# Ricardo-Ping/ChaoRec

Measured on AMD Instinct MI355X. Metric: GCN edges/sec + full-rank users-scored/sec, dim=64, higher is better.
Workload: dtype f32

## Files before the change

### chaorec_amd/csrc/score_prefilter.hpp

```cpp
#pragma once

typedef __bf16 bf16x8 __attribute__((ext_vector_type(8)));

union Frag16 {
  uint4 u;
  bf16x8 v;
};

__device__ __forceinline__ uint32_t bf16_rne_bits(float f) {
  const uint32_t b = __float_as_uint(f);
  return (b + 0x7FFFu + ((b >> 16) & 1u)) >> 16;
}
__device__ __forceinline__ float bf16_ceil_pos(float x) {
  const uint32_t b = __float_as_uint(x);
  return __uint_as_float(((b >> 16) + ((b & 0xFFFFu) ? 1u : 0u)) << 16);
}
__device__ __forceinline__ uint32_t bf16_pack2(float lo, float hi) {
  return bf16_rne_bits(lo) | (bf16_rne_bits(hi) << 16);
}
__device__ __forceinline__ uint4 bf16_pack8(const float4 a, const float4 b) {
  return make_uint4(bf16_pack2(a.x, a.y), bf16_pack2(a.z, a.w), bf16_pack2(b.x, b.y), bf16_pack2(b.z, b.w));
}

template <int CTRL, int ROW_MASK, bool BOUND>
// ... 819 lines not shown
      int tt = split + (kSweepStage * s0 + i) * splits;
      if (tt >= n_tiles) tt = n_tiles - 1;
      pre[p] = make_uint4(0u, 0u, 0u, 0u);
      if (i < kSweepStage) pre[p] = P.packed[(size_t)tt * (FR * 64) + w];
    }
  };
  auto stash = [&](int buf) __attribute__((always_inline)) {
#pragma unroll
    for (int p = 0; p < PER; ++p) {
      const int e = threadIdx.x + p * 64 * kSweepWaves;
      if (e < kSweepStage * FR * 64) (&stage[buf][0][0])[e] = pre[p];
    }
  };
  const int n_mine = split < n_tiles ? (n_tiles - split + splits - 1) / splits : 0;
  const int n_stages = (n_mine + kSweepStage - 1) / kSweepStage;
  int next_nb = 0;
  if (n_stages > 0) {
    fetch(0);
    stash(0);
    if constexpr (CLS) next_nb = __builtin_amdgcn_readfirstlane(__float_as_int(pre_nb));
  }
  __syncthreads();
  int s0 = 0;
  while (s0 < n_stages) {
    if constexpr (CLS) {
      cur_nb = next_nb;
      rescale(__int_as_float(cur_nb));
    }
    for (;;) {
      const int buf = s0 & 1;
      if (s0 + 1 < n_stages) fetch(s0 + 1);
#pragma unroll
      for (int i = 0; i < kSweepStage; ++i) {
        const int seq = kSweepStage * s0 + i;
        const int t = split + seq * splits;
        if (t < n_tiles) {
          uint4 a[FR];
#pragma unroll
          for (int q = 0; q < FR; ++q) a[q] = stage[buf][i][q * 64 + lane];
          consume(a, t, seq);
        }
      }
      if (s0 + 1 < n_stages) {
        stash(buf ^ 1);
        if constexpr (CLS) next_nb = __builtin_amdgcn_readfirstlane(__float_as_int(pre_nb));
      }
      __syncthreads();
      ++s0;
      if (s0 >= n_stages) break;
      if constexpr (CLS) {
        if (next_nb != cur_nb) break;
      }
    }
  }
#pragma unroll
  for (int b = 0; b < UB; ++b) {
    if constexpr (kSweepPark > 0) {
#pragma unroll
      for (int c0 = 0; c0 < kSweepPark; c0 += 4) {
        if (c0 < cnt[b]) {
          uint4 q;
          q.x = park_s[wv][b][c0][lane], q.y = park_s[wv][b][c0 + 1][lane];
          q.z = park_s[wv][b][c0 + 2][lane], q.w = park_s[wv][b][c0 + 3][lane];
          *reinterpret_cast<uint4 *>(mine[b] + c0) = q;
        }
      }
    }
    const int64_t uc = (ublock0 + b) * 32 + ur;
    if (uc < n_act) {
      const int64_t u = P.user_map ? (int64_t)P.user_map[uc] : uc;
      P.cand_cnt[((size_t)split * P.n_users + u) * 2 + h] = cnt[b];
    }
  }
}

template <int D>
__device__ __forceinline__ float exact_score(const float *__restrict__ urow, const float *__restrict__ irow) {
  float acc = 0.f;
  const float4 *i0 = reinterpret_cast<const float4 *>(irow), *i1 = reinterpret_cast<const float4 *>(irow + D / 2);
  const float4 *u0 = reinterpret_cast<const float4 *>(urow), *u1 = reinterpret_cast<const float4 *>(urow + D / 2);
#pragma unroll
  for (int q = 0; q < D / 8; ++q) {
    const float4 a = i0[q], b = i1[q], x = u0[q], y = u1[q];
    acc = __fmaf_rn(x.x, a.x, acc);
    acc = __fmaf_rn(y.x, b.x, acc);
    acc = __fmaf_rn(x.y, a.y, acc);
    acc = __fmaf_rn(y.y, b.y, acc);
    acc = __fmaf_rn(x.z, a.z, acc);
    acc = __fmaf_rn(y.z, b.z, acc);
    acc = __fmaf_rn(x.w, a.w, acc);
    acc = __fmaf_rn(y.w, b.w, acc);
  }
  return acc;
}

__device__ __forceinline__ float dpp_quad_rot(float v) {
  return __int_as_float(__builtin_amdgcn_update_dpp(0, __float_as_int(v), 0x93 , 0xF, 0xF, false));
}
template <int D>
__device__ __forceinline__ float exact_scores_64(const float *__restrict__ item_emb, int64_t i0, int64_t n_items,
                                                 const float (&ua)[D / 8], const float (&ub)[D / 8], int lane) {
  constexpr int G = 4, CPI = 16, SEG = D / 8;
  const int l = lane % G, g = lane / G;
  auto load_rows = [&](float (&a)[SEG], float (&b)[SEG], int pass) __attribute__((always_inline)) {
    const int64_t item = min(i0 + pass * CPI + g, n_items - 1);
    const float *row = item_emb + (size_t)item * D + 4 * l;
#pragma unroll
    for (int i = 0; i < SEG; i += 4) {
      const float4 x = reinterpret_cast<const float4 *>(row + 4 * i)[0];
      const float4 y = reinterpret_cast<const float4 *>(row + D / 2 + 4 * i)[0];
      a[i] = x.x, a[i + 1] = x.y, a[i + 2] = x.z, a[i + 3] = x.w;
      b[i] = y.x, b[i + 1] = y.y, b[i + 2] = y.z, b[i + 3] = y.w;
    }
  };
  float sc = 0.f;
  float a[SEG], b[SEG];
  load_rows(a, b, 0);
#pragma unroll
  for (int it = 0; it < G; ++it) {
    float ca[SEG], cb[SEG];
#pragma unroll
    for (int i = 0; i < SEG; ++i) ca[i] = a[i], cb[i] = b[i];
    if (it + 1 < G) load_rows(a, b, it + 1);
    float acc = 0.f;
#pragma unroll
    for (int seg = 0; seg < SEG; ++seg) {
      float t = acc;
#pragma unroll
      for (int i = 4 * (seg / G); i < 4 * (seg / G) + 4; ++i) {
        t = __fmaf_rn(ua[i], ca[i], t);
        t = __fmaf_rn(ub[i], cb[i], t);
      }
      if (l == seg % G) acc = t;
      if (seg + 1 < SEG) {
        const float nx = dpp_quad_rot(acc);
        if (l == (seg + 1) % G) acc = nx;
      }
    }
    const float moved = __shfl(acc, (lane % CPI) * G + G - 1, 64);
    if (lane / CPI == it) sc = moved;
  }
  return sc;
}

template <int NR>
__device__ __forceinline__ uint64_t kth_largest_key(const uint64_t (&k)[NR], int rank) {
  uint32_t T = 0;
  for (int bit = 31; bit >= 0; --bit) {
    const uint32_t candv = T | (1u << bit);
    int c = 0;
#pragma unroll
    for (int r = 0; r < NR; ++r) c += __popcll(__ballot(k[r] != 0ull && (uint32_t)(k[r] >> 32) >= candv));
    if (c >= rank) T = candv;
  }
  int gt = 0, eq = 0;
#pragma unroll
  for (int r = 0; r < NR; ++r) {
    gt += __popcll(__ballot(k[r] != 0ull && (uint32_t)(k[r] >> 32) > T));
    eq += __popcll(__ballot(k[r] != 0ull && (uint32_t)(k[r] >> 32) == T));
  }
  const int need = rank - gt;
  uint32_t L = 0;
  if (eq > need) {
    for (int bit = 31; bit >= 0; --bit) {
      const uint32_t candv = L | (1u << bit);
      int c = 0;
#pragma unroll
      for (int r = 0; r < NR; ++r)
        c += __popcll(__ballot(k[r] != 0ull && (uint32_t)(k[r] >> 32) == T && (uint32_t)k[r] >= candv));
      if (c >= need) L = candv;
    }
  }
  return ((uint64_t)T << 32) | (uint64_t)L;
}

__device__ __forceinline__ void sort64_desc(uint64_t &e, int lane) {
#pragma unroll
  for (int k = 2; k <= 64; k <<= 1) {
#pragma unroll
    for (int j = k >> 1; j > 0; j >>= 1) {
      const uint64_t p = shfl_xor_u64(e, j);
      const bool lower = (lane & j) == 0;
      const bool desc = (k == 64) ? true : ((lane & k) == 0);
      const uint64_t mx = e > p ? e : p, mn = e > p ? p : e;
      e = (lower == desc) ? mx : mn;
    }
  }
}

constexpr int kPfHistLds = 1024;
constexpr int kPfSelHist = 128;


__device__ __forceinline__ int wave_scan_add(int x) {
  x += dpp_or0<0x111, 0xF, true>(x);
  x += dpp_or0<0x112, 0xF, true>(x);
  x += dpp_or0<0x114, 0xF, true>(x);
  x += dpp_or0<0x118, 0xF, true>(x);
  x += dpp_or0<0x142, 0xA, false>(x);
  x += dpp_or0<0x143, 0xC, false>(x);
  return x;
}
__device__ __forceinline__ int wave_scan_max(int x) {
  x = max(x, dpp_or0<0x111, 0xF, true>(x));
  x = max(x, dpp_or0<0x112, 0xF, true>(x));
  x = max(x, dpp_or0<0x114, 0xF, true>(x));
  x = max(x, dpp_or0<0x118, 0xF, true>(x));
  x = max(x, dpp_or0<0x142, 0xA, false>(x));
  x = max(x, dpp_or0<0x143, 0xC, false>(x));
  return x;
}
__device__ __forceinline__ float dpp_prev_lane(float v) {
  return __int_as_float(__builtin_amdgcn_update_dpp(0, __float_as_int(v), 0x111 , 0xF, 0xF, false));
}

__device__ __forceinline__ uint32_t lane_select(uint32_t a, uint32_t b, uint64_t m) {
  uint32_t r;
  asm("v_cndmask_b32 %0, %1, %2, %3" : "=v"(r) : "v"(a), "v"(b), "s"(m));
  return r;
}
__device__ __forceinline__ uint64_t lane_select64(uint64_t a, uint64_t b, uint64_t m) {
  return ((uint64_t)lane_select((uint32_t)(a >> 32), (uint32_t)(b >> 32), m) << 32) | lane_select((uint32_t)a, (uint32_t)b, m);
}
struct PermAddr {
  int x0, x1, x2, x3, x4, x5, rev;
  template <int I>
  __device__ __forceinline__ int x() const {
    if constexpr (I == 0) return x0;
    else if constexpr (I == 1) return x1;
    else if constexpr (I == 2) return x2;
    else if constexpr (I == 3) return x3;
    else if constexpr (I == 4) return x4;
    else return x5;
  }
};
__device__ __forceinline__ PermAddr perm_addr(int lane) {
  PermAddr a;
  a.x0 = (lane ^ 1) << 2, a.x1 = (lane ^ 2) << 2, a.x2 = (lane ^ 4) << 2, a.x3 = (lane ^ 8) << 2;
  a.x4 = (lane ^ 16) << 2, a.x5 = (lane ^ 32) << 2, a.rev = (63 - lane) << 2;
  return a;
}
__device__ __forceinline__ uint64_t permute64(uint64_t v, int addr) {
  const uint32_t lo = (uint32_t)__builtin_amdgcn_ds_bpermute(addr, (int)(uint32_t)v);
  const uint32_t hi = (uint32_t)__builtin_amdgcn_ds_bpermute(addr, (int)(uint32_t)(v >> 32));
  return ((uint64_t)hi << 32) | lo;
}
__device__ __forceinline__ void compare_exchange(uint64_t &e, uint64_t p, uint64_t keepmax) {
  const uint64_t gt = __ballot(p > e);
  e = lane_select64(e, p, ~(gt ^ keepmax));
}
constexpr uint64_t keepmax_mask(int k, int j, bool all_desc) {
  uint64_t m = 0;
  for (int lane = 0; lane < 64; ++lane) {
    const bool lower = (lane & j) == 0, desc = all_desc || (lane & k) == 0;
    if (lower == desc) m |= 1ull << lane;
  }
  return m;
}
template <int LOGJ>
__device__ __forceinline__ void merge_stages(uint64_t &e, const PermAddr &pa) {
  compare_exchange(e, permute64(e, pa.template x<LOGJ>()), keepmax_mask(64, 1 << LOGJ, true));
  if constexpr (LOGJ > 0) merge_stages<LOGJ - 1>(e, pa);
}
template <int LOGK, int LOGJ>
__device__ __forceinline__ void sort_stages(uint64_t &e, const PermAddr &pa) {
  compare_exchange(e, permute64(e, pa.template x<LOGJ>()), keepmax_mask(1 << LOGK, 1 << LOGJ, LOGK == 6));
  if constexpr (LOGJ > 0) sort_stages<LOGK, LOGJ - 1>(e, pa);
  else if constexpr (LOGK < 6) sort_stages<LOGK + 1, LOGK>(e, pa);
}
__device__ __forceinline__ void sort64_keys(uint64_t &e, const PermAddr &pa) { sort_stages<1, 0>(e, pa); }
__device__ __forceinline__ void merge128_keys(uint64_t &e0, uint64_t &e1, const PermAddr &pa) {
  const uint64_t r = permute64(e1, pa.rev);
  const uint64_t gt = __ballot(r > e0);
  const uint64_t hi = lane_select64(e0, r, gt), lo = lane_select64(r, e0, gt);
  e0 = hi;
  e1 = lo;
  merge_stages<5>(e0, pa);
  merge_stages<5>(e1, pa);
}
__device__ __forceinline__ void merge_block_keys(uint64_t &e0, uint64_t &e1, uint64_t b, const PermAddr &pa) {
  sort64_keys(b, pa);
  const uint64_t r = permute64(b, pa.rev);
  e1 = lane_select64(e1, r, __ballot(r > e1));
  merge_stages<5>(e1, pa);
  merge128_keys(e0, e1, pa);
}

__device__ __forceinline__ void take_block_keys(uint64_t &e0, uint64_t &e1, int &blocks, uint64_t cur, const PermAddr &pa) {
  if (blocks == 0) {
    sort64_keys(cur, pa);
    e0 = cur;
  } else if (blocks == 1) {
    sort64_keys(cur, pa);
    uint64_t a = e0, b = cur;
    merge128_keys(a, b, pa);
    e0 = a, e1 = b;
  } else {
    uint64_t a = e0, b = e1;
    merge_block_keys(a, b, cur, pa);
    e0 = a, e1 = b;
  }
  ++blocks;
}
__device__ __forceinline__ uint64_t key_of_rank(uint64_t e0, uint64_t e1, int rank) {
  const uint32_t lo0 = (uint32_t)__builtin_amdgcn_readlane((int)(uint32_t)e0, rank & 63);
  const uint32_t hi0 = (uint32_t)__builtin_amdgcn_readlane((int)(uint32_t)(e0 >> 32), rank & 63);
  const uint32_t lo1 = (uint32_t)__builtin_amdgcn_readlane((int)(uint32_t)e1, rank & 63);
  const uint32_t hi1 = (uint32_t)__builtin_amdgcn_readlane((int)(uint32_t)(e1 >> 32), rank & 63);
  return rank < 64 ? (((uint64_t)hi0 << 32) | lo0) : (((uint64_t)hi1 << 32) | lo1);
}

#ifndef CHAOREC_SEL_G
#define CHAOREC_SEL_G 4
#endif
constexpr int kSelG = CHAOREC_SEL_G;
template <int D>
__device__ __forceinline__ float chain_block(const float *__restrict__ item_emb, const uint32_t *cand_s, int base, int n_cand,
                                             const float (&ua)[D / (2 * kSelG)], const float (&ub)[D / (2 * kSelG)], int lane) {
  constexpr int G = kSelG, CPI = 64 / G, SEG = D / (2 * G);
  const int l = lane % G, g = lane / G;
  auto load_rows = [&](float (&a)[SEG], float (&b)[SEG], int c) __attribute__((always_inline)) {
    const float *row = item_emb + (size_t)cand_s[c] * D;
#pragma unroll
    for (int i = 0; i < SEG; i += 4) {
      const float4 x = reinterpret_cast<const float4 *>(row + SEG * l)[i / 4];
      const float4 y = reinterpret_cast<const float4 *>(row + D / 2 + SEG * l)[i / 4];
      a[i] = x.x, a[i + 1] = x.y, a[i + 2] = x.z, a[i + 3] = x.w;
      b[i] = y.x, b[i + 1] = y.y, b[i + 2] = y.z, b[i + 3] = y.w;
    }
  };
  float sc = 0.f;
  float a[SEG], b[SEG];
#pragma unroll
  for (int i = 0; i < SEG; ++i) a[i] = b[i] = 0.f;
  if (base + g < n_cand) load_rows(a, b, base + g);
  for (int it = 0; it < G; ++it) {
    if (base + it * CPI >= n_cand) break;
    float ca[SEG], cb[SEG];
#pragma unroll
    for (int i = 0; i < SEG; ++i) ca[i] = a[i], cb[i] = b[i];
    const int cn = base + (it + 1) * CPI + g;
    if (it + 1 < G && cn < n_cand) load_rows(a, b, cn);
    float acc = 0.f;
#pragma unroll
    for (int seg = 0; seg < G; ++seg) {
      float t = acc;
#pragma unroll
      for (int i = 0; i < SEG; ++i) {
        t = __fmaf_rn(ua[i], ca[i], t);
        t = __fmaf_rn(ub[i], cb[i], t);
      }
      if (l == seg) acc = t;
      if (seg + 1 < G) {
        const float nx = dpp_prev_lane(acc);
        if (l == seg + 1) acc = nx;
      }
    }
    const float moved = __shfl(acc, (lane % CPI) * G + G - 1, 64);
    if (lane / CPI == it) sc = moved;
  }
  return sc;
}

template <int D, int MAXC>
__device__ __forceinline__ void select_user(const PrefArgs &P, const int64_t u, int lane, int2 *meta_s, uint32_t *cand_s,
                                            uint32_t *hist_s, float *score_s) {
  const int K = P.K;
  const int n_lists = 2 * P.splits;
  const PermAddr pa = perm_addr(lane);

  const int listidx = (int)(((int64_t)(lane >> 1) * P.n_users + u) * 2 + (lane & 1));
  int c = 0;
  if (lane < n_lists) c = P.cand_cnt[listidx];
  float ua[D / (2 * kSelG)], ub[D / (2 * kSelG)];
  {
    const float *urow = P.user_emb + (size_t)u * D + (D / (2 * kSelG)) * (lane % kSelG);
#pragma unroll
    for (int i = 0; i < D / (2 * kSelG); i += 4) {
      const float4 x = reinterpret_cast<const float4 *>(urow)[i / 4], y = reinterpret_cast<const float4 *>(urow + D / 2)[i / 4];
      ua[i] = x.x, ua[i + 1] = x.y, ua[i + 2] = x.z, ua[i + 3] = x.w;
      ub[i] = y.x, ub[i + 1] = y.y, ub[i + 2] = y.z, ub[i + 3] = y.w;
    }
  }
  int64_t hb = 0, he = 0;
  if (P.hist_rowptr) {
    hb = P.hist_rowptr[u];
    he = P.hist_rowptr[u + 1];
  }
  const int deg = (int)(he - hb);
  const bool hist_lds = deg <= kPfSelHist;
  const float theta = P.theta[u];
  const bool overflow = __any(c > kPfCap);
  const int incl = wave_scan_add(c);
  const int total = __builtin_amdgcn_readlane(incl, 63);
  int why = overflow ? 1 : (total > MAXC ? 3 : 0);
  int n_cand = 0;
  if (why == 0) {
    int *owner_s = reinterpret_cast<int *>(score_s);
#pragma unroll 1
    for (int i = lane; i < total; i += 64) owner_s[i] = 0;
    meta_s[lane] = make_int2(incl - c, listidx);
    if (hist_lds) {
#pragma unroll 1
      for (int i = lane; i < deg; i += 64) hist_s[i] = (uint32_t)P.hist_col[hb + i];
    }
    __builtin_amdgcn_wave_barrier();
    if (c > 0) owner_s[incl - c] = lane + 1;
    __builtin_amdgcn_wave_barrier();
    int owner_carry = 0;
#pragma unroll 1
    for (int base = 0; base < total; base += 64) {
      const int e = base + lane;
      int own = e < total ? owner_s[e] : 0;
      own = max(wave_scan_max(own), owner_carry);
      owner_carry = __builtin_amdgcn_readlane(own, 63);
      uint32_t bits = 0, j0 = 0;
      if (e < total) {
        const int list = own - 1;
        const int2 m = meta_s[list];
        const uint32_t raw = P.cand[(size_t)m.y * kPfCap + (e - m.x)];
        bits = raw & 0xFFFFu;
        j0 = ((uint32_t)(list >> 1) + (raw >> 16) * (uint32_t)P.splits) * 32u + 4u * (uint32_t)(list & 1);
      }
      if (__any(bits != 0u && j0 + 32u > (uint32_t)P.n_items)) {
#pragma unroll 1
        for (int reg = 0; reg < 16; ++reg)
          if (j0 + (uint32_t)((reg & 3) + 8 * (reg >> 2)) >= (uint32_t)P.n_items) bits &= ~(1u << (15 - reg));
      }
      const int pc = __popc(bits);
      const int ex = wave_scan_add(pc);
      int slot = n_cand + ex - pc;
#pragma unroll 1
      while (__any(bits != 0u)) {
        if (bits) {
          const int bit = 31 - __clz(bits);
          bits &= ~(1u << bit);
          const int reg = 15 - bit;
          if (slot < MAXC) cand_s[slot] = j0 + (uint32_t)((reg & 3) + 8 * (reg >> 2));
          ++slot;
        }
      }
      n_cand += __builtin_amdgcn_readlane(ex, 63);
    }
    if (n_cand > MAXC) why = 3;
    __builtin_amdgcn_wave_barrier();
    if (P.perm && why == 0) {
#pragma unroll 1
      for (int i = lane; i < n_cand; i += 64) cand_s[i] = (uint32_t)P.perm[cand_s[i]];
      __builtin_amdgcn_wave_barrier();
    }
  }
  uint64_t e0 = 0ull, e1 = 0ull;
  if (why == 0) {
    auto in_hist = [&](uint32_t item) -> bool {
      int lo = 0, hi = deg;
      while (lo < hi) {
        const int mid = (lo + hi) >> 1;
        const uint32_t hv = hist_lds ? hist_s[mid] : (uint32_t)P.hist_col[hb + mid];
        if (hv < item) lo = mid + 1; else hi = mid;
      }
      return lo < deg && (hist_lds ? hist_s[lo] : (uint32_t)P.hist_col[hb + lo]) == item;
    };
    const uint32_t mord = f32_to_ord(P.mask_value);
    int valid = 0, above = 0, blocks = 0;
#pragma unroll 1
    for (int base = 0; base < n_cand; base += 64) {
      const float sc = chain_block<D>(P.item_emb, cand_s, base, n_cand, ua, ub, lane);
      const int idx = base + lane;
      uint64_t cur = 0ull;
      if (idx < n_cand) {
        const uint32_t item = cand_s[idx];
        if (deg == 0 || !in_hist(item)) cur = make_key(sc, item);
      }
      valid += __popcll(__ballot(cur != 0ull));
      above += __popcll(__ballot(cur != 0ull && (uint32_t)(cur >> 32) > mord));
      take_block_keys(e0, e1, blocks, cur, pa);
    }
    int n_keys = valid;
    if (deg > 0 && above < K) {
#pragma unroll 1
      for (int i0 = 0; i0 < deg; i0 += 64) {
        const int i = i0 + lane;
        take_block_keys(e0, e1, blocks, i < deg ? make_key(P.mask_value, hist_lds ? hist_s[i] : (uint32_t)P.hist_col[hb + i]) : 0ull, pa);
      }
      n_keys = valid + deg;
    }
    if (n_keys < K) why = 2;
    if (why == 0) {
      const uint64_t kth = key_of_rank(e0, e1, K - 1);
      if (kth == 0ull || !(ord_to_f32((uint32_t)(kth >> 32)) > theta)) why = 4;
      if (why == 0 && P.hint_out) {
        const int want = min(max(P.hint_rank, K), 128);
        const uint64_t hk = key_of_rank(e0, e1, min(want, n_keys) - 1);
        float t = nextafterf(ord_to_f32((uint32_t)(hk >> 32)), -INFINITY);
        if (n_keys < want) {
          const float s_k = ord_to_f32((uint32_t)(kth >> 32)), s_last = ord_to_f32((uint32_t)(hk >> 32));
          const float s_top = ord_to_f32((uint32_t)(key_of_rank(e0, e1, 0) >> 32));
          const float slope = n_keys > K ? (s_k - s_last) / (float)(n_keys - K) : (s_top - s_k) / (float)max(K - 1, 1);
          t -= slope * (float)(want - n_keys);
        }
        if (lane == 0) P.hint_out[u] = t;
      }
    }
  }
  if (lane == 0) {
    P.fail[u] = why;
    P.n_cand[u] = n_cand;
    if (why != 0) {
      if (P.retry_cnt) P.retry_list[atomicAdd(P.retry_cnt, 1)] = (int)u;
      else if (why == 3 && MAXC < kPfMaxCandWide && P.wide_cnt && n_cand <= kPfMaxCandWide && total <= kPfMaxCandWide)
        P.wide_list[atomicAdd(P.wide_cnt, 1)] = (int)u;
      else if ((why == 1 || why == 3) && P.reth_cnt) P.reth_list[atomicAdd(P.reth_cnt, 1)] = (int)u;
      else P.fb_list[atomicAdd(P.fb_cnt, 1)] = (int)u;
    }
  }
  if (why == 0 && lane < K) {
    const uint32_t item = 0xFFFFFFFFu - (uint32_t)(e0 & 0xFFFFFFFFull);
    P.out_idx[(size_t)u * K + lane] = (int64_t)item + P.id_offset;
    P.out_val[(size_t)u * K + lane] = ord_to_f32((uint32_t)(e0 >> 32));
  }
}

#ifndef CHAOREC_SEL_WAVES
#define CHAOREC_SEL_WAVES 4
#endif
template <int D, int MAXC>
__global__ __launch_bounds__(64, D > 64 ? 3 : (MAXC <= 512 ? CHAOREC_SEL_WAVES : 3)) void score_select_kernel_pf(const PrefArgs P) {
  __shared__ int2 meta_s[64];
  __shared__ uint32_t cand_s[MAXC];
  __shared__ uint32_t hist_s[kPfSelHist];
  __shared__ float score_s[MAXC];
  const int64_t n_act = P.n_active ? (int64_t)*P.n_active : P.n_users;
  if (n_act <= P.min_active) return;
#pragma unroll 1
  for (int64_t i = blockIdx.x; i < n_act; i += gridDim.x) {
    const int64_t u = P.user_map ? (int64_t)P.user_map[i] : i;
    int lane = threadIdx.x;
    asm volatile("" : "+v"(lane));
    select_user<D, MAXC>(P, u, lane, meta_s, cand_s, hist_s, score_s);
    __builtin_amdgcn_wave_barrier();
  }
}

constexpr int kPfRethTarget = 256;

template <int D>
__device__ __forceinline__ void rethreshold_user(const PrefArgs &P, const int64_t u, int lane, int2 *meta_s, uint32_t *cand_s,
                                                 uint32_t *hist_s, float *score_s) {
  constexpr int MAXC = kPfMaxCandWide;
  const int K = P.K;
  const int n_lists = 2 * P.splits;
  const PermAddr pa = perm_addr(lane);
  const int listidx = (int)(((int64_t)(lane >> 1) * P.n_users + u) * 2 + (lane & 1));
  int c_all = 0;
  if (lane < n_lists) c_all = P.cand_cnt[listidx];
  const int c = min(c_all, kPfCap);
  float ua[D / (2 * kSelG)], ub[D / (2 * kSelG)];
  {
    const float *urow = P.user_emb + (size_t)u * D + (D / (2 * kSelG)) * (lane % kSelG);
#pragma unroll
    for (int i = 0; i < D / (2 * kSelG); i += 4) {
      const float4 x = reinterpret_cast<const float4 *>(urow)[i / 4], y = reinterpret_cast<const float4 *>(urow + D / 2)[i / 4];
      ua[i] = x.x, ua[i + 1] = x.y, ua[i + 2] = x.z, ua[i + 3] = x.w;
      ub[i] = y.x, ub[i + 1] = y.y, ub[i + 2] = y.z, ub[i + 3] = y.w;
    }
  }
  int64_t hb = 0, he = 0;
  if (P.hist_rowptr) {
    hb = P.hist_rowptr[u];
    he = P.hist_rowptr[u + 1];
  }
  const int deg = (int)(he - hb);
  const bool hist_lds = deg <= kPfSelHist;
  const int incl = wave_scan_add(c);
  const int stored = __builtin_amdgcn_readlane(incl, 63);
  const int counted = __builtin_amdgcn_readlane(wave_scan_add(c_all), 63);
  const int used = min(stored, MAXC);
  int *owner_s = reinterpret_cast<int *>(score_s);
#pragma unroll 1
  for (int i = lane; i < used; i += 64) owner_s[i] = 0;
  meta_s[lane] = make_int2(incl - c, listidx);
  if (hist_lds) {
#pragma unroll 1
    for (int i = lane; i < deg; i += 64) hist_s[i] = (uint32_t)P.hist_col[hb + i];
  }
  __builtin_amdgcn_wave_barrier();
  if (c > 0 && incl - c < used) owner_s[incl - c] = lane + 1;
  __builtin_amdgcn_wave_barrier();
  int n_raw = 0, owner_carry = 0;
#pragma unroll 1
  for (int base = 0; base < used; base += 64) {
    const int e = base + lane;
    int own = e < used ? owner_s[e] : 0;
    own = max(wave_scan_max(own), owner_carry);
    owner_carry = __builtin_amdgcn_readlane(own, 63);
    uint32_t bits = 0, j0 = 0;
    if (e < used) {
      const int list = own - 1;
      const int2 m = meta_s[list];
      const uint32_t raw = P.cand[(size_t)m.y * kPfCap + (e - m.x)];
      bits = raw & 0xFFFFu;
      j0 = ((uint32_t)(list >> 1) + (raw >> 16) * (uint32_t)P.splits) * 32u + 4u * (uint32_t)(list & 1);
    }
    if (__any(bits != 0u && j0 + 32u > (uint32_t)P.n_items)) {
#pragma unroll 1
      for (int reg = 0; reg < 16; ++reg)
        if (j0 + (uint32_t)((reg & 3) + 8 * (reg >> 2)) >= (uint32_t)P.n_items) bits &= ~(1u << (15 - reg));
    }
    const int pc = __popc(bits);
    const int ex = wave_scan_add(pc);
    int slot = n_raw + ex - pc;
#pragma unroll 1
    while (__any(bits != 0u)) {
      if (bits) {
        const int bit = 31 - __clz(bits);
        bits &= ~(1u << bit);
        const int reg = 15 - bit;
        if (slot < MAXC) cand_s[slot] = j0 + (uint32_t)((reg & 3) + 8 * (reg >> 2));
        ++slot;
      }
    }
    n_raw += __builtin_amdgcn_readlane(ex, 63);
  }
  const int n_cand = min(n_raw, MAXC);
  __builtin_amdgcn_wave_barrier();
  if (P.perm) {
#pragma unroll 1
    for (int i = lane; i < n_cand; i += 64) cand_s[i] = (uint32_t)P.perm[cand_s[i]];
    __builtin_amdgcn_wave_barrier();
  }
  auto in_hist = [&](uint32_t item) -> bool {
    int lo = 0, hi = deg;
    while (lo < hi) {
      const int mid = (lo + hi) >> 1;
      const uint32_t hv = hist_lds ? hist_s[mid] : (uint32_t)P.hist_col[hb + mid];
      if (hv < item) lo = mid + 1; else hi = mid;
    }
    return lo < deg && (hist_lds ? hist_s[lo] : (uint32_t)P.hist_col[hb + lo]) == item;
  };
  uint64_t e0 = 0ull, e1 = 0ull;
  int valid = 0, blocks = 0;
#pragma unroll 1
  for (int base = 0; base < n_cand; base += 64) {
    const float sc = chain_block<D>(P.item_emb, cand_s, base, n_cand, ua, ub, lane);
    const int idx = base + lane;
    uint64_t cur = 0ull;
    if (idx < n_cand) {
      const uint32_t item = cand_s[idx];
      if (deg == 0 || !in_hist(item)) cur = make_key(sc, item);
    }
    valid += __popcll(__ballot(cur != 0ull));
    take_block_keys(e0, e1, blocks, cur, pa);
  }
  bool queued = false;
  if (valid >= K && n_cand > 0) {
    const float scale = ((float)counted / (float)used) * ((float)n_raw / (float)n_cand);
    int r = (int)ceilf((float)kPfRethTarget / scale);
    r = min(min(max(r, K + 6), 128), valid);
    if ((float)r * scale <= 0.9f * (float)kPfMaxCandWide) {
      const uint64_t rk = key_of_rank(e0, e1, r - 1);
      if (lane == 0) {
        P.tau_sum[u] = nextafterf(ord_to_f32((uint32_t)(rk >> 32)), -INFINITY);
        P.rt2_list[atomicAdd(P.rt2_cnt, 1)] = (int)u;
      }
      queued = true;
    }
  }
  if (!queued && lane == 0) P.fb_list[atomicAdd(P.fb_cnt, 1)] = (int)u;
}

template <int D>
__global__ __launch_bounds__(64, 3) void score_rethreshold_kernel(const PrefArgs P) {
  __shared__ int2 meta_s[64];
  __shared__ uint32_t cand_s[kPfMaxCandWide];
  __shared__ uint32_t hist_s[kPfSelHist];
  __shared__ float score_s[kPfMaxCandWide];
  const int64_t n_act = (int64_t)*P.reth_cnt;
#pragma unroll 1
  for (int64_t i = blockIdx.x; i < n_act; i += gridDim.x) {
    const int64_t u = (int64_t)P.reth_list[i];
    int lane = threadIdx.x;
    asm volatile("" : "+v"(lane));
    rethreshold_user<D>(P, u, lane, meta_s, cand_s, hist_s, score_s);
    __builtin_amdgcn_wave_barrier();
  }
}

constexpr int kExThreads = 1024;
template <int D>
constexpr int ex_threads() { return D <= 64 ? kExThreads : kExThreads / 2; }
constexpr int kExPer = 2;
constexpr int kExSlices = 8;

template <int NK>
__device__ __forceinline__ uint64_t wave_select_topk(const uint64_t (&key)[NK], uint64_t bk, int K, uint64_t *stage) {
  const int lane = threadIdx.x & 63;
  int have = __popcll(__ballot(bk != 0ull));
#pragma unroll
  for (int j = 0; j < NK; ++j) have += __popcll(__ballot(key[j] != 0ull));
  const int want = min(K, have);
  uint32_t T = 0;
  for (int bit = 31; bit >= 0; --bit) {
    const uint32_t cand = T | (1u << bit);
    int c = __popcll(__ballot(bk != 0ull && (uint32_t)(bk >> 32) >= cand));
#pragma unroll
    for (int j = 0; j < NK; ++j) c += __popcll(__ballot(key[j] != 0ull && (uint32_t)(key[j] >> 32) >= cand));
    if (c >= want) T = cand;
  }
  int gt = __popcll(__ballot(bk != 0ull && (uint32_t)(bk >> 32) > T));
  int eq = __popcll(__ballot(bk != 0ull && (uint32_t)(bk >> 32) == T));
#pragma unroll
  for (int j = 0; j < NK; ++j) {
    gt += __popcll(__ballot(key[j] != 0ull && (uint32_t)(key[j] >> 32) > T));
    eq += __popcll(__ballot(key[j] != 0ull && (uint32_t)(key[j] >> 32) == T));
  }
  const int need = want - gt;
  uint32_t L = 0;
  if (eq > need) {
    for (int bit = 31; bit >= 0; --bit) {
      const uint32_t cand = L | (1u << bit);
      int c = __popcll(__ballot(bk != 0ull && (uint32_t)(bk >> 32) == T && (uint32_t)bk >= cand));
#pragma unroll
      for (int j = 0; j < NK; ++j)
        c += __popcll(__ballot(key[j] != 0ull && (uint32_t)(key[j] >> 32) == T && (uint32_t)key[j] >= cand));
      if (c >= need) L = cand;
    }
  }
  const uint64_t thr = ((uint64_t)T << 32) | (uint64_t)L;
  stage[lane] = 0ull;
  __builtin_amdgcn_wave_barrier();
  int base = 0;
  {
    const bool w = bk != 0ull && bk >= thr;
    const unsigned long long m = __ballot(w);
    if (w) stage[__builtin_amdgcn_mbcnt_hi((unsigned)(m >> 32), __builtin_amdgcn_mbcnt_lo((unsigned)m, 0))] = bk;
    base = __popcll(m);
  }
#pragma unroll
  for (int j = 0; j < NK; ++j) {
    const bool w = key[j] != 0ull && key[j] >= thr;
    const unsigned long long m = __ballot(w);
    if (w) stage[base + __builtin_amdgcn_mbcnt_hi((unsigned)(m >> 32), __builtin_amdgcn_mbcnt_lo((unsigned)m, 0))] = key[j];
    base += __popcll(m);
  }
  __builtin_amdgcn_wave_barrier();
  const uint64_t out = stage[lane];
  __builtin_amdgcn_wave_barrier();
  return out;
}

__device__ __forceinline__ uint64_t merge_top64(uint64_t a, uint64_t b, int lane) {
  const uint64_t r = shfl_u64(b, 63 - lane);
  uint64_t m = a > r ? a : r;
#pragma unroll
  for (int j = 32; j > 0; j >>= 1) {
    const uint64_t p = shfl_xor_u64(m, j);
    const uint64_t mx = m > p ? m : p, mn = m > p ? p : m;
    m = (lane & j) == 0 ? mx : mn;
  }
  return m;
}

template <int D>
__global__ __launch_bounds__(ex_threads<D>()) void score_exact_user_kernel(const PrefArgs P) {
  constexpr int kExThreads = ex_threads<D>();
  constexpr int NW = kExThreads / 64;
  __shared__ uint64_t stage[NW][64];
  __shared__ uint32_t hist_s[kPfHistLds];
  __shared__ int last;
  const int tid = threadIdx.x, lane = tid & 63, wave = tid >> 6;
  const int K = P.K;
  const int n_fb = *P.fb_cnt;
  int n_rt = P.retry_list ? *(P.retry_list_cnt) : 0;
  if (n_rt > P.small_retry) n_rt = 0;
  if (P.counters_out && blockIdx.x == 0 && tid == 0) {
    P.counters_out[0] = P.retry_list ? *(P.retry_list_cnt) : 0;
    P.counters_out[1] = n_fb;
    P.counters_out[2] = P.wide_cnt ? *P.wide_cnt : 0;
    P.counters_out[3] = n_rt;
  }
  const int64_t per_slice = (P.n_items + kExSlices - 1) / kExSlices;
  for (int w = blockIdx.x + P.fb_skip * kExSlices; w < (n_fb + n_rt) * kExSlices; w += gridDim.x) {
    const int qi = w / kExSlices, slice = w % kExSlices;
    const int64_t u = qi < n_fb ? P.fb_list[qi] : P.retry_list[qi - n_fb];
    const float *urow = P.user_emb + (size_t)u * D;
    int64_t hb = 0, he = 0;
    if (P.hist_rowptr) {
      hb = P.hist_rowptr[u];
      he = P.hist_rowptr[u + 1];
    }
    const int deg = (int)(he - hb);
    const bool hist_lds = deg <= kPfHistLds;
    __syncthreads();
    constexpr int HR = kPfHistLds / kExThreads;
    uint32_t hreg[HR];
#pragma unroll
    for (int q = 0; q < HR; ++q) hreg[q] = (hist_lds && tid + q * kExThreads < deg) ? (uint32_t)P.hist_col[hb + tid + q * kExThreads] : 0u;
    bool hist_ready = false;
    const int64_t i_begin = (int64_t)slice * per_slice, i_end = min(P.n_items, i_begin + per_slice);
    float ua[D / 8], ub[D / 8];
#pragma unroll
    for (int i = 0; i < D / 8; ++i) {
      ua[i] = urow[16 * (i / 4) + 4 * (lane & 3) + (i & 3)];
      ub[i] = urow[D / 2 + 16 * (i / 4) + 4 * (lane & 3) + (i & 3)];
    }
    uint64_t bk = 0ull;
    for (int64_t c0 = i_begin; c0 < i_end; c0 += (int64_t)kExThreads * kExPer) {
      uint64_t key[kExPer];
      float sxs[kExPer];
#pragma unroll
      for (int j = 0; j < kExPer; ++j) {
        const int64_t it0 = c0 + 64 * wave + (int64_t)kExThreads * j;
        sxs[j] = 0.f;
        if (it0 < i_end) sxs[j] = exact_scores_64<D>(P.item_emb, it0, P.n_items, ua, ub, lane);
      }
      if (!hist_ready) {
#pragma unroll
        for (int q = 0; q < HR; ++q)
          if (tid + q * kExThreads < deg) hist_s[tid + q * kExThreads] = hreg[q];
        __syncthreads();
        hist_ready = true;
      }
#pragma unroll
      for (int j = 0; j < kExPer; ++j) {
        const int64_t it0 = c0 + 64 * wave + (int64_t)kExThreads * j;
        const int64_t it = it0 + lane;
        key[j] = 0ull;
        if (it0 < i_end) {
          const float sx = sxs[j];
          if (it < i_end) {
            const uint32_t item = (uint32_t)it;
            int lo = 0, hi = deg;
            while (lo < hi) {
              const int mid = (lo + hi) >> 1;
              const uint32_t hv = hist_lds ? hist_s[mid] : (uint32_t)P.hist_col[hb + mid];
              if (hv < item) lo = mid + 1; else hi = mid;
            }
            const bool masked = lo < deg && (hist_lds ? hist_s[lo] : (uint32_t)P.hist_col[hb + lo]) == item;
            key[j] = make_key(masked ? P.mask_value : sx, item);
          }
        }
      }
      bk = wave_select_topk<kExPer>(key, bk, kMaxK, stage[wave]);
    }
    sort64_desc(bk, lane);
    stage[wave][lane] = bk;
    __syncthreads();
#pragma unroll
    for (int half = NW / 2; half >= 1; half >>= 1) {
      uint64_t mine = 0ull;
      if (wave < half) mine = merge_top64(stage[wave][lane], stage[wave + half][lane], lane);
      __syncthreads();
      if (wave < half) stage[wave][lane] = mine;
      __syncthreads();
    }
    uint64_t *part = P.fb_partial + (size_t)qi * kExSlices * kMaxK;
    if (wave == 0) {
      part[slice * kMaxK + lane] = stage[0][lane];
      __threadfence();
      if (lane == 0) last = atomicAdd(P.fb_done + qi, 1) == kExSlices - 1 ? 1 : 0;
    }
    __syncthreads();
    if (last && wave == 0) {
      __threadfence();
      uint64_t sl[kExSlices];
#pragma unroll
      for (int j = 0; j < kExSlices; ++j) sl[j] = __builtin_nontemporal_load(part + j * kMaxK + lane);
      uint64_t e = sl[0];
#pragma unroll
      for (int j = 1; j < kExSlices; ++j) e = merge_top64(e, sl[j], lane);
      if (lane < K) {
        const uint32_t item = 0xFFFFFFFFu - (uint32_t)(e & 0xFFFFFFFFull);
        P.out_idx[(size_t)u * K + lane] = (int64_t)item + P.id_offset;
        P.out_val[(size_t)u * K + lane] = ord_to_f32((uint32_t)(e >> 32));
      }
      if (P.hint_out) {
        const uint32_t o31 = (uint32_t)__shfl((int)(uint32_t)(e >> 32), 31, 64), o63 = (uint32_t)__shfl((int)(uint32_t)(e >> 32), 63, 64);
        const uint64_t ek = shfl_u64(e, K - 1);
        float t = nextafterf(ord_to_f32((uint32_t)(ek >> 32)), -INFINITY);
        if (shfl_u64(e, 63) != 0ull) {
          const float s31 = ord_to_f32(o31), s63 = ord_to_f32(o63);
          t = fminf(t, s63 - (s31 - s63));
        }
        if (lane == 0) P.hint_out[u] = t;
      }
    }
  }
}

__global__ __launch_bounds__(256) void score_prefilter_stats_kernel(const int *__restrict__ fail,
                                                                    const int *__restrict__ cand_cnt,
                                                                    const int *__restrict__ n_cand, int64_t n_users,
                                                                    int splits, unsigned long long *__restrict__ out,
                                                                    const int *__restrict__ rt2_cnt) {
  const int64_t u = (int64_t)blockIdx.x * blockDim.x + threadIdx.x;
  if (u == 0 && rt2_cnt) out[9] = (unsigned long long)*rt2_cnt;
  if (u >= n_users) return;
  int mx = 0;
  if (cand_cnt) {
    for (int l = 0; l < 2 * splits; ++l) mx = max(mx, cand_cnt[((size_t)(l >> 1) * n_users + u) * 2 + (l & 1)]);
  } else {
    mx = n_cand[u];
  }
  if (fail[u]) {
    atomicAdd(out + 0, 1ull);
    atomicAdd(out + 3 + min(fail[u], 5), 1ull);
  }
  atomicAdd(out + 1, (unsigned long long)n_cand[u]);
  atomicMax(out + 2, (unsigned long long)mx);
  atomicAdd(out + 3, 1ull);
}
```

Before: 16.00 billion.

## Score two candidate blocks per round with packed f32x2 FMAs in selection

Candidate scoring in the per-user top-K selection now processes 128 candidates per round instead of 64. Two item rows are interleaved into f32x2 registers so packed FMAs compute two dot products at once. The two sorted key blocks are then merged through a new take_round_keys helper. This aims to halve the scalar FMA issue count and raise memory-level parallelism in the prefilter scoring loop, at the cost of higher register pressure and added v_pk_mov shuffles.

Result: no change. 16.08 billion (median of 3 runs) (+0.5%).

```diff
diff --git a/chaorec_amd/csrc/score_prefilter.hpp b/chaorec_amd/csrc/score_prefilter.hpp
--- a/chaorec_amd/csrc/score_prefilter.hpp
+++ b/chaorec_amd/csrc/score_prefilter.hpp
@@ -1145,6 +1145,27 @@
   }
   ++blocks;
 }
+__device__ __forceinline__ void take_round_keys(uint64_t &e0, uint64_t &e1, int &blocks, const uint64_t (&cur)[2], bool second,
+                                                const PermAddr &pa) {
+  if (blocks == 0) {
+    uint64_t a = cur[0], b = 0ull;
+    sort64_keys(a, pa);
+    if (second) {
+      b = cur[1];
+      sort64_keys(b, pa);
+      merge128_keys(a, b, pa);
+    }
+    e0 = a, e1 = b;
+  } else {
+#pragma unroll 1
+    for (int s = 0; s < (second ? 2 : 1); ++s) {
+      uint64_t a = e0, b = e1;
+      merge_block_keys(a, b, s ? cur[1] : cur[0], pa);
+      e0 = a, e1 = b;
+    }
+  }
+  blocks += second ? 2 : 1;
+}
 __device__ __forceinline__ uint64_t key_of_rank(uint64_t e0, uint64_t e1, int rank) {
   const uint32_t lo0 = (uint32_t)__builtin_amdgcn_readlane((int)(uint32_t)e0, rank & 63);
   const uint32_t hi0 = (uint32_t)__builtin_amdgcn_readlane((int)(uint32_t)(e0 >> 32), rank & 63);
@@ -1203,6 +1224,93 @@
     if (lane / CPI == it) sc = moved;
   }
   return sc;
+}
+
+#ifndef CHAOREC_SEL_PACKED
+#define CHAOREC_SEL_PACKED 1
+#endif
+template <int D>
+constexpr bool sel_packed() { return CHAOREC_SEL_PACKED != 0 && D <= 64 && kSelG % 2 == 0; }
+typedef float f32x2 __attribute__((ext_vector_type(2)));
+
+__device__ __forceinline__ f32x2 pk_pair_lo(f32x2 a, f32x2 b) {
+  f32x2 r;
+  asm("v_pk_mov_b32 %0, %1, %2 op_sel:[0,0] op_sel_hi:[0,0]" : "=v"(r) : "v"(a), "v"(b));
+  return r;
+}
+__device__ __forceinline__ f32x2 pk_pair_hi(f32x2 a, f32x2 b) {
+  f32x2 r;
+  asm("v_pk_mov_b32 %0, %1, %2 op_sel:[1,1] op_sel_hi:[1,1]" : "=v"(r) : "v"(a), "v"(b));
+  return r;
+}
+
+template <int D>
+__device__ __forceinline__ void chain_round(const float *__restrict__ item_emb, const uint32_t *cand_s, int base, int n_cand,
+                                            const float (&ua)[D / (2 * kSelG)], const float (&ub)[D / (2 * kSelG)], int lane,
+                                            float (&sc)[2]) {
+  if constexpr (!sel_packed<D>()) {
+    sc[0] = chain_block<D>(item_emb, cand_s, base, n_cand, ua, ub, lane);
+    sc[1] = 0.f;
+    if (base + 64 < n_cand) sc[1] = chain_block<D>(item_emb, cand_s, base + 64, n_cand, ua, ub, lane);
+  } else {
+    constexpr int G = kSelG, CPI = 64 / G, SEG = D / (2 * G), H = SEG / 2;
+    static_assert(SEG % 4 == 0, "whole float4 pieces");
+    const int l = lane % G, g = lane / G;
+    auto load_rows = [&](f32x2 (&a)[H], f32x2 (&b)[H], int c) __attribute__((always_inline)) {
+      const float *row = item_emb + (size_t)cand_s[min(c, n_cand - 1)] * D;
+#pragma unroll
+      for (int i = 0; i < H; i += 2) {
+        const float4 x = reinterpret_cast<const float4 *>(row + SEG * l)[i / 2];
+        const float4 y = reinterpret_cast<const float4 *>(row + D / 2 + SEG * l)[i / 2];
+        a[i] = f32x2{x.x, x.y}, a[i + 1] = f32x2{x.z, x.w};
+        b[i] = f32x2{y.x, y.y}, b[i + 1] = f32x2{y.z, y.w};
+      }
+    };
+    f32x2 u2a[H], u2b[H];
+#pragma unroll
+    for (int i = 0; i < H; ++i) u2a[i] = f32x2{ua[2 * i], ua[2 * i + 1]}, u2b[i] = f32x2{ub[2 * i], ub[2 * i + 1]};
+    sc[0] = sc[1] = 0.f;
+    f32x2 a0[H], b0[H], a1[H], b1[H];
+    load_rows(a0, b0, base + g);
+    load_rows(a1, b1, base + CPI + g);
+#pragma unroll
+    for (int p = 0; p < G; ++p) {
+      f32x2 ca[SEG], cb[SEG];
+#pragma unroll
+      for (int i = 0; i < H; ++i) {
+        ca[2 * i] = pk_pair_lo(a0[i], a1[i]), ca[2 * i + 1] = pk_pair_hi(a0[i], a1[i]);
+        cb[2 * i] = pk_pair_lo(b0[i], b1[i]), cb[2 * i + 1] = pk_pair_hi(b0[i], b1[i]);
+      }
+      const bool more = p + 1 < G && base + (2 * p + 2) * CPI < n_cand;
+      if (more) {
+        load_rows(a0, b0, base + (2 * p + 2) * CPI + g);
+        load_rows(a1, b1, base + (2 * p + 3) * CPI + g);
+      }
+      f32x2 acc = f32x2{0.f, 0.f};
+#pragma unroll
+      for (int seg = 0; seg < G; ++seg) {
+        f32x2 t = acc;
+#pragma unroll
+        for (int i = 0; i < H; ++i) {
+          t = __builtin_elementwise_fma(__builtin_shufflevector(u2a[i], u2a[i], 0, 0), ca[2 * i], t);
+          t = __builtin_elementwise_fma(__builtin_shufflevector(u2b[i], u2b[i], 0, 0), cb[2 * i], t);
+          t = __builtin_elementwise_fma(__builtin_shufflevector(u2a[i], u2a[i], 1, 1), ca[2 * i + 1], t);
+          t = __builtin_elementwise_fma(__builtin_shufflevector(u2b[i], u2b[i], 1, 1), cb[2 * i + 1], t);
+        }
+        if (l == seg) acc = t;
+        if (seg + 1 < G) {
+          const f32x2 nx = f32x2{dpp_prev_lane(acc.x), dpp_prev_lane(acc.y)};
+          if (l == seg + 1) acc = nx;
+        }
+      }
+      const int src = (lane % CPI) * G + G - 1;
+      const float m0 = __shfl(acc.x, src, 64), m1 = __shfl(acc.y, src, 64);
+      float &dst = sc[(2 * p) / G];
+      if (lane / CPI == (2 * p) % G) dst = m0;
+      if (lane / CPI == (2 * p + 1) % G) dst = m1;
+      if (!more) break;
+    }
+  }
 }
 
 template <int D, int MAXC>
@@ -1307,17 +1415,22 @@
     const uint32_t mord = f32_to_ord(P.mask_value);
     int valid = 0, above = 0, blocks = 0;
 #pragma unroll 1
-    for (int base = 0; base < n_cand; base += 64) {
-      const float sc = chain_block<D>(P.item_emb, cand_s, base, n_cand, ua, ub, lane);
-      const int idx = base + lane;
-      uint64_t cur = 0ull;
-      if (idx < n_cand) {
-        const uint32_t item = cand_s[idx];
-        if (deg == 0 || !in_hist(item)) cur = make_key(sc, item);
-      }
-      valid += __popcll(__ballot(cur != 0ull));
-      above += __popcll(__ballot(cur != 0ull && (uint32_t)(cur >> 32) > mord));
-      take_block_keys(e0, e1, blocks, cur, pa);
+    for (int base = 0; base < n_cand; base += 128) {
+      float sc[2];
+      chain_round<D>(P.item_emb, cand_s, base, n_cand, ua, ub, lane, sc);
+      uint64_t cur[2] = {0ull, 0ull};
+#pragma unroll
+      for (int s = 0; s < 2; ++s) {
+        const int idx = base + 64 * s + lane;
+        if (idx < n_cand) {
+          const uint32_t item = cand_s[idx];
+          if (deg == 0 || !in_hist(item)) cur[s] = make_key(sc[s], item);
+        }
+      }
+      valid += __popcll(__ballot(cur[0] != 0ull)) + __popcll(__ballot(cur[1] != 0ull));
+      above += __popcll(__ballot(cur[0] != 0ull && (uint32_t)(cur[0] >> 32) > mord)) +
+               __popcll(__ballot(cur[1] != 0ull && (uint32_t)(cur[1] >> 32) > mord));
+      take_round_keys(e0, e1, blocks, cur, base + 64 < n_cand, pa);
     }
     int n_keys = valid;
     if (deg > 0 && above < K) {
@@ -1484,16 +1597,20 @@
   uint64_t e0 = 0ull, e1 = 0ull;
   int valid = 0, blocks = 0;
 #pragma unroll 1
-  for (int base = 0; base < n_cand; base += 64) {
-    const float sc = chain_block<D>(P.item_emb, cand_s, base, n_cand, ua, ub, lane);
-    const int idx = base + lane;
-    uint64_t cur = 0ull;
-    if (idx < n_cand) {
-      const uint32_t item = cand_s[idx];
-      if (deg == 0 || !in_hist(item)) cur = make_key(sc, item);
-    }
-    valid += __popcll(__ballot(cur != 0ull));
-    take_block_keys(e0, e1, blocks, cur, pa);
+  for (int base = 0; base < n_cand; base += 128) {
+    float sc[2];
+    chain_round<D>(P.item_emb, cand_s, base, n_cand, ua, ub, lane, sc);
+    uint64_t cur[2] = {0ull, 0ull};
+#pragma unroll
+    for (int s = 0; s < 2; ++s) {
+      const int idx = base + 64 * s + lane;
+      if (idx < n_cand) {
+        const uint32_t item = cand_s[idx];
+        if (deg == 0 || !in_hist(item)) cur[s] = make_key(sc[s], item);
+      }
+    }
+    valid += __popcll(__ballot(cur[0] != 0ull)) + __popcll(__ballot(cur[1] != 0ull));
+    take_round_keys(e0, e1, blocks, cur, base + 64 < n_cand, pa);
   }
   bool queued = false;
   if (valid >= K && n_cand > 0) {
```
